# DeepBlender/DeepDenoiser

Measured on AMD Instinct MI355X. Metric: train tiles/sec (128x128x32ch U-Net KPCN), higher is better.
Workload: dtype bf16; 1 GPU; BASELINE config 2: U-Net [64,96,128]x4 + 5x5 KernelPrediction + 3-scale MultiScalePrediction, 32-channel render-pass stack, 128x128 tiles, full training step (fwd+SMAPE loss+bwd+Adam); global_batch=128, parallelism=dp1, hipgraph=True, inputs=resident in HBM

## Files before the change

deepdenoiser_amd/csrc/dd_convt.hip:

```cpp
#include "dd_common.h"

namespace {

struct CtP {
  const void* x; const void* y; const void* w; void* out; float* dw; float* db; const float* bias;
  int ldx, ldy, ldo;
  int cin, cout, cinv, coutv;
  int n_pad, k_pad;
  int B, H, W, tiles_x, tiles_y, nwg;
  int relu;
  int co_off, cout_total;
};

typedef __attribute__((address_space(3))) s16x4_t* ct_tr_ptr;
typedef uint32_t ct_u32x4 __attribute__((ext_vector_type(4)));
typedef uint32_t ct_u32x2 __attribute__((ext_vector_type(2)));

constexpr int CT_T = 8;
constexpr int CT_X_SLICE = CT_T * CT_T * DD_LDS_ROW;
constexpr int CT_X_BYTES = 2 * CT_X_SLICE;
constexpr int CT_Y_BYTES = 4 * CT_T * CT_T * DD_LDS_ROW;
constexpr int CT_BWD_BUF = CT_Y_BYTES + CT_X_BYTES;
constexpr int CT_FWD_BUF = CT_X_BYTES;

__device__ __forceinline__ void ct_dma_1k(const void* gptr, unsigned lds_addr) {
  asm volatile("s_mov_b32 m0, %1\n\ts_nop 0\n\tglobal_load_lds_dwordx4 %0, off" : : "v"(gptr), "s"(lds_addr) : "memory");
}
__device__ __forceinline__ uint4 ct_lds16(unsigned off) {
  const ct_u32x4 v = *reinterpret_cast<const __attribute__((address_space(3))) ct_u32x4*>(off);
  return uint4{v[0], v[1], v[2], v[3]};
}
__device__ __forceinline__ uint2 ct_lds8(unsigned off) {
  const ct_u32x2 v = *reinterpret_cast<const __attribute__((address_space(3))) ct_u32x2*>(off);
  return uint2{v[0], v[1]};
}
__device__ __forceinline__ uint4 ct_tr_pair(unsigned a0, unsigned a1) {
  const s16x4_t lo = __builtin_amdgcn_ds_read_tr16_b64_v4i16(reinterpret_cast<ct_tr_ptr>(a0));
  const s16x4_t hi = __builtin_amdgcn_ds_read_tr16_b64_v4i16(reinterpret_cast<ct_tr_ptr>(a1));
  const uint2 l2 = __builtin_bit_cast(uint2, lo), h2 = __builtin_bit_cast(uint2, hi);
  return uint4{l2.x, l2.y, h2.x, h2.y};
}

struct CtTile { int b, i0, j0; bool live; };
__device__ __forceinline__ CtTile ct_tile(const CtP& a, int tile, int total, int th = CT_T) {
  CtTile t;
  t.live = tile < total;
  const int u = t.live ? tile : 0, per_img = a.tiles_x * a.tiles_y;
  t.b = u / per_img;
  const int rem = u - t.b * per_img, ty = rem / a.tiles_x;
  t.i0 = ty * th; t.j0 = (rem - ty * a.tiles_x) * CT_T;
  return t;
}
template <int TH = CT_T>
__device__ __forceinline__ void ct_dma_x(const CtP& a, const CtTile& t, int xc, unsigned lds, int lane) {
  const int r = lane >> 3, ls = (lane & 7) ^ r;
  const int sx = xc / TH, row = xc % TH, ch = sx * 64 + ls * 8;
  const bool ok = t.live && ch < a.cinv && t.i0 + row < a.H && t.j0 + r < a.W;
  const char* src = reinterpret_cast<const char*>(a.x) + (((long)t.b * a.H + t.i0 + row) * a.W + t.j0 + r) * a.ldx * 2 + ch * 2;
  ct_dma_1k(ok ? src : reinterpret_cast<const char*>(&dd_zero16_v), lds + xc * 1024);
}
template <int NSD>
__device__ __forceinline__ void ct_dma_y(const CtP& a, const CtTile& t, int c, unsigned lds, int lane) {
  const int r = lane >> 3, ls = (lane & 7) ^ r;
  const int sd = c / (32 / NSD), cc = c % (32 / NSD);
  const int row = cc >> 1, col = (cc & 1) * 8 + r, ch = sd * 64 + ls * 8;
  const int gy = 2 * t.i0 + row, gx = 2 * t.j0 + col;
  const bool ok = t.live && ch < a.coutv && gy < 2 * a.H && gx < 2 * a.W;
  const char* src = reinterpret_cast<const char*>(a.y) + (((long)t.b * 2 * a.H + gy) * 2 * a.W + gx) * a.ldy * 2 + (a.co_off + ch) * 2;
  ct_dma_1k(ok ? src : reinterpret_cast<const char*>(&dd_zero16_v), lds + c * 1024);
}

template <typename T, int KC>
__global__ __launch_bounds__(512) void convt_fwd_kernel(const CtP a) {
  extern __shared__ __attribute__((aligned(1024))) char smem[];
  constexpr int NTW = 3;
  const int tid = threadIdx.x, lane = tid & 63, wave = __builtin_amdgcn_readfirstlane(tid >> 6);
  const int li = lane & 15, q = lane >> 4;
  const unsigned lds_base = (unsigned)(uintptr_t)(__attribute__((address_space(3))) char*)smem;
  const int total = a.B * a.tiles_x * a.tiles_y;
  const int ntiles = (4 * a.cout) >> 4;
  const T* Wp = reinterpret_cast<const T*>(a.w);
  const T* zw = reinterpret_cast<const T*>(&dd_zero16_v);
  uint4 wf[NTW][KC];
  float bv[NTW][4];
  int och[NTW], opix[NTW];
  bool nt_ok[NTW];
#pragma unroll
  for (int u = 0; u < NTW; ++u) {
    const int nt = wave + 8 * u;
    nt_ok[u] = nt < ntiles;
    const int nrow = nt * 16 + li;
#pragma unroll
    for (int kc = 0; kc < KC; ++kc) {
      const int k0 = kc * 32 + q * 8;
      const bool ok = nt_ok[u] && nrow < a.n_pad && k0 < a.k_pad;
      wf[u][kc] = *reinterpret_cast<const uint4*>(ok ? Wp + (long)nrow * a.k_pad + k0 : zw);
    }
    const int n4 = nt * 16 + q * 4;
// ... 32 lines not shown
#pragma unroll
        for (int u = 0; u < NTW; ++u) acc[g][u] = mma16<T>(wf[u][kc], f, acc[g][u]);
      }
    const int jj = cur.j0 + (li & 7);
#pragma unroll
    for (int g = 0; g < 4; ++g) {
      const int ii = cur.i0 + 2 * g + (li >> 3);
      const bool ok = ii < a.H && jj < a.W;
      const long p0 = ((long)cur.b * 2 * a.H + 2 * ii) * 2 * a.W + 2 * jj;
#pragma unroll
      for (int u = 0; u < NTW; ++u) {
        f32x4_t v = acc[g][u];
        if (a.relu) { v[0] = fmaxf(v[0], 0.f); v[1] = fmaxf(v[1], 0.f); v[2] = fmaxf(v[2], 0.f); v[3] = fmaxf(v[3], 0.f); }
        uint2 o2;
        o2.x = pack2<T>(v[0], v[1]);
        o2.y = pack2<T>(v[2], v[3]);
        if (ok && nt_ok[u]) *reinterpret_cast<uint2*>(Y + (p0 + opix[u]) * a.ldy + och[u]) = o2;
      }
    }
    cur = nxt;
  }
}

template <typename T> __device__ __forceinline__ void ct_mma_inplace(f32x4_t& acc, const uint4& a, const uint4& b);
template <> __device__ __forceinline__ void ct_mma_inplace<bf16_t>(f32x4_t& acc, const uint4& a, const uint4& b) {
  const ct_u32x4 av = {a.x, a.y, a.z, a.w}, bv = {b.x, b.y, b.z, b.w};
  asm volatile("v_mfma_f32_16x16x32_bf16 %0, %1, %2, %0" : "+v"(acc) : "v"(av), "v"(bv));
}
template <> __device__ __forceinline__ void ct_mma_inplace<f16_t>(f32x4_t& acc, const uint4& a, const uint4& b) {
  const ct_u32x4 av = {a.x, a.y, a.z, a.w}, bv = {b.x, b.y, b.z, b.w};
  asm volatile("v_mfma_f32_16x16x32_f16 %0, %1, %2, %0" : "+v"(acc) : "v"(av), "v"(bv));
}

template <typename T, int NSD, bool MASK, bool ACCUM>
__global__ __launch_bounds__(512) void convt_bwd_kernel(const CtP a) {
  extern __shared__ __attribute__((aligned(1024))) char smem[];
  constexpr int TH = CT_T / NSD, NG = TH / 2, KC = 2 * NSD, JW = 2 * NSD, KS = TH / 4;
  constexpr int Y_SLICE = CT_Y_BYTES / NSD, X_SLICE = CT_T * TH * DD_LDS_ROW, BUF = CT_Y_BYTES + 2 * X_SLICE;
  const int tid = threadIdx.x, lane = tid & 63, wave = __builtin_amdgcn_readfirstlane(tid >> 6);
  const int li = lane & 15, q = lane >> 4;
  const unsigned lds_base = (unsigned)(uintptr_t)(__attribute__((address_space(3))) char*)smem;
  const int total = a.B * a.tiles_x * a.tiles_y;

  const bool d_active = wave * 16 < a.cin;
  uint4 wf[4][KC];
  {
    const T* Wd = reinterpret_cast<const T*>(a.w);
    const T* zw = reinterpret_cast<const T*>(&dd_zero16_v);
    const int ci_row = wave * 16 + li;
#pragma unroll
    for (int t = 0; t < 4; ++t)
#pragma unroll
      for (int kc = 0; kc < KC; ++kc) {
        const int k0 = kc * 32 + q * 8;
        const bool ok = ci_row < a.n_pad && k0 < a.coutv && a.co_off + k0 < a.k_pad;
        wf[t][kc] = *reinterpret_cast<const uint4*>(ok ? Wd + ((long)t * a.n_pad + ci_row) * a.k_pad + a.co_off + k0 : zw);
      }
  }
  unsigned db[4];
#pragma unroll
  for (int t = 0; t < 4; ++t) {
    const int pd = (2 * (li >> 3) + (t >> 1)) * 16 + 2 * (li & 7) + (t & 1);
    db[t] = lds_base + pd * DD_LDS_ROW + ((q ^ (pd & 7)) << 4);
  }
  const unsigned mb = lds_base + CT_Y_BYTES + (wave >> 2) * X_SLICE + li * DD_LDS_ROW + ((((wave & 3) * 2 + (q >> 1)) ^ (li & 7)) << 4) + (q & 1) * 8;
  const int c4 = wave * 16 + q * 4;
  T* __restrict__ DX = reinterpret_cast<T*>(a.out);

  const int tw = wave & 3, h = wave >> 2;
  const bool w_active = h * JW * 16 < a.cout;
  const int nci = (a.cin + 15) >> 4;
  unsigned yb[2], xb[2];
  {
    const int t16 = lane & 15, gq = lane >> 4, sub = t16 & 3;
#pragma unroll
    for (int hh = 0; hh < 2; ++hh) {
      const int col = (t16 >> 2) + 4 * hh;
      const int pd = (2 * gq + (tw >> 1)) * 16 + 2 * col + (tw & 1), px = gq * 8 + col;
      yb[hh] = lds_base + ((h * JW) >> 2) * Y_SLICE + pd * DD_LDS_ROW + (((((h * JW) & 3) * 2 + (sub >> 1)) ^ (pd & 7)) << 4) + (sub & 1) * 8;
      xb[hh] = lds_base + CT_Y_BYTES + px * DD_LDS_ROW + (((sub >> 1) ^ (px & 7)) << 4) + (sub & 1) * 8;
    }
  }
  f32x4_t wacc[JW][8];
#pragma unroll
  for (int j = 0; j < JW; ++j)
#pragma unroll
    for (int i = 0; i < 8; ++i) wacc[j][i] = f32x4_t{0.f, 0.f, 0.f, 0.f};
  float bsum[JW];
#pragma unroll
  for (int j = 0; j < JW; ++j) bsum[j] = 0.f;

  auto dma_tile = [&](const CtTile& t, unsigned buf) {
#pragma unroll
    for (int k = 0; k < 4; ++k) ct_dma_y<NSD>(a, t, k * 8 + wave, buf, lane);
    ct_dma_x<TH>(a, t, wave, buf + CT_Y_BYTES, lane);
    if (NSD == 1) ct_dma_x<TH>(a, t, wave + 8, buf + CT_Y_BYTES, lane);
  };
  constexpr int NPW = 5 + (NSD == 1 ? 1 : 0);
  CtTile cur = ct_tile(a, blockIdx.x, total, TH);
  dma_tile(cur, lds_base);
  int sel = 0;
  for (int tile = blockIdx.x; tile < total; tile += a.nwg, sel ^= 1) {
    __builtin_amdgcn_s_waitcnt(0x0F70);
    __syncthreads();
    const CtTile nxt = ct_tile(a, tile + a.nwg, total, TH);
    const int jj = cur.j0 + (li & 7);
    const bool ch_ok = c4 < a.cinv && jj < a.W;
    ct_u32x2 oldr[NG];
    if (ACCUM) {
#pragma unroll
      for (int g = 0; g < NG; ++g) {
        const int ii = cur.i0 + 2 * g + (li >> 3);
        const bool ok = d_active && ch_ok && ii < a.H;
        const void* op = ok ? static_cast<const void*>(DX + (((long)cur.b * a.H + ii) * a.W + jj) * a.ldo + c4) : static_cast<const void*>(&dd_zero16_v);
        asm volatile("global_load_dwordx2 %0, %1, off ; dd_accum_request" : "=v"(oldr[g]) : "v"(op) : "memory");
      }
    }
    dma_tile(nxt, lds_base + (sel ^ 1) * BUF);
    const unsigned bt = sel * BUF;
    if (d_active) {
      f32x4_t acc[NG];
      uint2 mv[NG], oldv[NG];
#pragma unroll
      for (int g = 0; g < NG; ++g) {
        acc[g] = f32x4_t{0.f, 0.f, 0.f, 0.f};
        if (MASK) mv[g] = ct_lds8(bt + mb + g * 16 * DD_LDS_ROW);
        oldv[g] = uint2{0u, 0u};
      }
#pragma unroll
      for (int t = 0; t < 4; ++t)
#pragma unroll
        for (int kc = 0; kc < KC; ++kc)
#pragma unroll
          for (int g = 0; g < NG; ++g) {
            const uint4 f = ct_lds16(bt + (db[t] ^ ((kc & 1) << 6)) + (kc >> 1) * Y_SLICE + g * 64 * DD_LDS_ROW);
            acc[g] = mma16<T>(wf[t][kc], f, acc[g]);
          }
      if (ACCUM) {
        static_assert(NG == 4 || NG == 2, "the wait below names every request register");
        if constexpr (NG == 4) {
          if constexpr (NPW == 6) asm volatile("s_waitcnt vmcnt(6) ; dd_accum_wait" : "+v"(oldr[0]), "+v"(oldr[1]), "+v"(oldr[2]), "+v"(oldr[3]));
          else asm volatile("s_waitcnt vmcnt(5) ; dd_accum_wait" : "+v"(oldr[0]), "+v"(oldr[1]), "+v"(oldr[2]), "+v"(oldr[3]));
        } else {
          if constexpr (NPW == 6) asm volatile("s_waitcnt vmcnt(6) ; dd_accum_wait" : "+v"(oldr[0]), "+v"(oldr[1]));
          else asm volatile("s_waitcnt vmcnt(5) ; dd_accum_wait" : "+v"(oldr[0]), "+v"(oldr[1]));
        }
#pragma unroll
        for (int g = 0; g < NG; ++g) oldv[g] = uint2{oldr[g][0], oldr[g][1]};
      }
#pragma unroll
      for (int g = 0; g < NG; ++g) {
        const int ii = cur.i0 + 2 * g + (li >> 3);
        uint2 o2;
        o2.x = pack2<T>(acc[g][0], acc[g][1]);
        o2.y = pack2<T>(acc[g][2], acc[g][3]);
        if (MASK) { o2.x = mask_bf16x2(o2.x, mv[g].x); o2.y = mask_bf16x2(o2.y, mv[g].y); }
        if (ACCUM) {
          float f8[8], g8[8];
          unpack8t<T>(uint4{o2.x, o2.y, 0u, 0u}, f8);
          unpack8t<T>(uint4{oldv[g].x, oldv[g].y, 0u, 0u}, g8);
          o2.x = pack2<T>(f8[0] + g8[0], f8[1] + g8[1]);
          o2.y = pack2<T>(f8[2] + g8[2], f8[3] + g8[3]);
        }
        if (ch_ok && ii < a.H) *reinterpret_cast<uint2*>(DX + (((long)cur.b * a.H + ii) * a.W + jj) * a.ldo + c4) = o2;
      }
    }
    if (w_active) {
#pragma unroll
      for (int s = 0; s < KS; ++s) {
        uint4 yf[JW];
#pragma unroll
        for (int j = 0; j < JW; ++j)
          yf[j] = ct_tr_pair(bt + (yb[0] ^ (j << 5)) + s * 128 * DD_LDS_ROW, bt + (yb[1] ^ (j << 5)) + s * 128 * DD_LDS_ROW);
#pragma unroll
        for (int i = 0; i < 8; ++i) {
          if (i >= nci) continue;
          const uint4 xf = ct_tr_pair(bt + (xb[0] ^ ((i & 3) << 5)) + (i >> 2) * X_SLICE + s * 32 * DD_LDS_ROW,
                                      bt + (xb[1] ^ ((i & 3) << 5)) + (i >> 2) * X_SLICE + s * 32 * DD_LDS_ROW);
#pragma unroll
          for (int j = 0; j < JW; ++j) ct_mma_inplace<T>(wacc[j][i], yf[j], xf);
        }
        if (a.db) {
#pragma unroll
          for (int j = 0; j < JW; ++j) {
            float f[8];
            unpack8t<T>(yf[j], f);
            bsum[j] += ((f[0] + f[1]) + (f[2] + f[3])) + ((f[4] + f[5]) + (f[6] + f[7]));
          }
        }
      }
    }
    cur = nxt;
  }
  asm volatile("s_nop 15\n\ts_nop 15" ::: "memory");
  dd_det_wait();
  if (w_active) {
#pragma unroll
    for (int j = 0; j < JW; ++j)
#pragma unroll
      for (int i = 0; i < 8; ++i) {
        const int ci = i * 16 + li;
        if (i >= nci || ci >= a.cin) continue;
#pragma unroll
        for (int e = 0; e < 4; ++e) {
          const int co = (h * JW + j) * 16 + q * 4 + e;
          if (co < a.cout) atomicAdd(a.dw + ((long)tw * a.cout_total + a.co_off + co) * a.cin + ci, wacc[j][i][e]);
// ... 19 lines not shown

static int ct_cus() {
  return dd_device_cus();
}

template <typename K>
static void ct_launch(K kernel, const CtP& p, size_t lds, hipStream_t stream) {
  dd_det_sync();
  dd_allow_max_lds(reinterpret_cast<const void*>(kernel));
  hipLaunchKernelGGL(kernel, dim3((unsigned)p.nwg), dim3(512), lds, stream, p);
}

static int ct_fill(CtP& p, const dd_convt_args* a, bool bwd) {
  const int th = CT_T;
  DD_REQUIRE(a && a->x && a->y && a->w, "dd_convt2x2: null pointer");
  DD_REQUIRE(a->dtype == DD_BF16 || a->dtype == DD_F16, "dd_convt2x2: dtype %d (bf16 / f16 storage only; f32 takes dd_conv_igemm / dd_conv_wgrad)", a->dtype);
  DD_REQUIRE(a->cin > 0 && a->cin <= 128 && a->cout > 0 && a->cout <= (bwd ? 128 : 96) && a->cout % 16 == 0,
             "dd_convt2x2: cin=%d cout=%d (cin <= 128; cout a multiple of 16, <= 96 forward / 128 backward)", a->cin, a->cout);
  const int cinv = (a->cin + 7) / 8 * 8, coutv = (a->cout + 7) / 8 * 8;
  DD_REQUIRE(a->ld_x % 8 == 0 && a->ld_y % 8 == 0 && cinv <= a->ld_x && coutv <= a->ld_y, "dd_convt2x2: ld_x=%d ld_y=%d must be multiples of 8 covering the channels", a->ld_x, a->ld_y);
  DD_REQUIRE(((uintptr_t)a->x % 16) == 0 && ((uintptr_t)a->y % 16) == 0 && ((uintptr_t)a->w % 16) == 0, "dd_convt2x2: x / y / w must be 16-byte aligned");
  DD_REQUIRE(a->B > 0 && a->H > 0 && a->W > 0 && (long)a->B * a->H * a->W * 4 < (1L << 31), "dd_convt2x2: empty or oversized grid");
  p.x = a->x; p.y = a->y; p.w = a->w; p.ldx = a->ld_x; p.ldy = a->ld_y;
  p.cin = a->cin; p.cout = a->cout; p.cinv = cinv; p.coutv = coutv; p.n_pad = a->n_pad; p.k_pad = a->k_pad;
  p.B = a->B; p.H = a->H; p.W = a->W;
  p.tiles_x = dd_ceil_div(a->W, CT_T); p.tiles_y = dd_ceil_div(a->H, th);
  const long total = (long)a->B * p.tiles_x * p.tiles_y;
  p.nwg = (int)(total < ct_cus() ? total : ct_cus());
  p.relu = a->relu;
  p.co_off = 0; p.cout_total = a->cout;
  return DD_OK;
}

}

extern "C" int dd_convt2x2_fwd(const dd_convt_args* a, dd_stream stream) {
  CtP p;
  if (int rc = ct_fill(p, a, false)) return rc;
  DD_REQUIRE(a->n_pad >= 4 * a->cout && a->k_pad >= a->cin && a->k_pad % 32 == 0 && a->k_pad <= 128, "dd_convt2x2_fwd: packed weights [n_pad=%d][k_pad=%d]", a->n_pad, a->k_pad);
  p.out = const_cast<void*>(a->y); p.bias = a->bias; p.dw = nullptr; p.db = nullptr; p.ldo = 0;
  hipStream_t s = reinterpret_cast<hipStream_t>(stream);
  const size_t lds = 2 * (size_t)CT_FWD_BUF;
  const int kc = a->k_pad / 32;
#define CT_FWD(T)                                                            \
  switch (kc) {                                                              \
    case 1: ct_launch(convt_fwd_kernel<T, 1>, p, lds, s); break;             \
    case 2: ct_launch(convt_fwd_kernel<T, 2>, p, lds, s); break;             \
    case 3: ct_launch(convt_fwd_kernel<T, 3>, p, lds, s); break;             \
    default: ct_launch(convt_fwd_kernel<T, 4>, p, lds, s); break;            \
  }
  if (a->dtype == DD_BF16) { CT_FWD(bf16_t) } else { CT_FWD(f16_t) }
#undef CT_FWD
  DD_LAUNCH_CHECK();
  return DD_OK;
}

extern "C" int dd_convt2x2_bwd(const dd_convt_args* a, dd_stream stream) {
  CtP p;
  if (int rc = ct_fill(p, a, true)) return rc;
  DD_REQUIRE(a->dx && a->dw, "dd_convt2x2_bwd: null gradient pointer");
  DD_REQUIRE(a->n_pad >= a->cin && a->k_pad >= a->cout && a->k_pad % 8 == 0, "dd_convt2x2_bwd: packed weights [4][n_pad=%d][k_pad=%d]", a->n_pad, a->k_pad);
  const int cinv = (a->cin + 7) / 8 * 8;
  DD_REQUIRE(a->ld_dx % 4 == 0 && cinv <= a->ld_dx && ((uintptr_t)a->dx % 8) == 0, "dd_convt2x2_bwd: ld_dx=%d / dx alignment", a->ld_dx);
  p.out = a->dx; p.ldo = a->ld_dx; p.dw = a->dw; p.db = a->db; p.bias = nullptr;
  hipStream_t s = reinterpret_cast<hipStream_t>(stream);
  const size_t lds = 2 * (size_t)CT_BWD_BUF;
#define CT_BWD_N(T, N, ACC)                                                                                \
  if (a->use_mask) { if (ACC) ct_launch(convt_bwd_kernel<T, N, true, true>, p, lds, s); else ct_launch(convt_bwd_kernel<T, N, true, false>, p, lds, s); } \
  else { if (ACC) ct_launch(convt_bwd_kernel<T, N, false, true>, p, lds, s); else ct_launch(convt_bwd_kernel<T, N, false, false>, p, lds, s); }
  for (int co_off = 0; co_off < a->cout; co_off += 64) {
    const int cb = a->cout - co_off < 64 ? a->cout - co_off : 64;
    p.co_off = co_off; p.cout = cb; p.coutv = (cb + 7) / 8 * 8; p.cout_total = a->cout;
    const bool acc = a->accumulate || co_off > 0;
    if (a->dtype == DD_BF16) { CT_BWD_N(bf16_t, 1, acc) } else { CT_BWD_N(f16_t, 1, acc) }
  }
#undef CT_BWD_N
  DD_LAUNCH_CHECK();
  return DD_OK;
}
```

deepdenoiser_amd/_lib.py:

```python

import ctypes as C
import os

_HERE = os.path.dirname(os.path.abspath(__file__))
LIB_PATH = os.environ.get("DD_LIB", os.path.join(_HERE, "libdd_hip.so"))

DD_F32, DD_BF16, DD_F16 = 0, 1, 2
IN_RELU, OUT_RELU, ACCUM, PIXSHUF, GATHER2X2 = 1, 2, 4, 8, 16
MAX_FEATURES, MAX_COMBINED = 32, 8
METRIC_SOURCES = MAX_FEATURES + MAX_COMBINED + 1

SYMBOLS = (
    "dd_version", "dd_last_error", "dd_pack_weights", "dd_pack_weights_batched", "dd_conv_igemm", "dd_conv_wgrad", "dd_colsum", "dd_colsum_segments",
    "dd_maxpool_fwd", "dd_maxpool_bwd", "dd_avgpool", "dd_prepare_feature", "dd_gather_input",
    "dd_kpcn_fwd", "dd_kpcn_bwd", "dd_kpcn_hidden_fwd", "dd_kpcn_hidden_bwd", "dd_compose_pack", "dd_compose_blend_fwd", "dd_compose_blend_bwd",
    "dd_compose_unpack_bwd", "dd_invert_std_fwd", "dd_invert_std_bwd", "dd_loss_head", "dd_adam_step",
    "dd_stitch", "dd_recombine", "dd_probe_tr16", "dd_masked_add", "dd_zero_stuff", "dd_zero_unstuff", "dd_convert_channels",
    "dd_augment", "dd_loss_mask_sums", "dd_crc32c", "dd_extract_tiles", "dd_compose_net_fwd", "dd_compose_net_bwd",
    "dd_kpcn_head_fwd", "dd_kpcn_head_bwd", "dd_kpcn_head_bwd_multi", "dd_assemble_input", "dd_assemble_input_frames", "dd_conv3x3_bwd", "dd_conv3x3_bwd_multi", "dd_convt2x2_fwd", "dd_convt2x2_bwd", "dd_conv3x3_ks",
    "dd_conv_pw_count", "dd_wgrad_pw_count", "dd_space_to_depth2", "dd_convt3_wgrad", "dd_compose_stream_plan", "dd_compose_bwd_scratch_bytes",
    "dd_loss_msssim_scratch_bytes", "dd_loss_msssim_fwd", "dd_loss_msssim_bwd", "dd_loss_msssim_values",
    "dd_loss_metrics_scratch_bytes", "dd_loss_metrics", "dd_loss_head_path_count",
)


class ConvT3WgradArgs(C.Structure):
    _fields_ = [("s", C.c_void_p), ("lds", C.c_int), ("cout", C.c_int), ("cp", C.c_int),
                ("x", C.c_void_p), ("ldx", C.c_int), ("cin", C.c_int),
                ("dk", C.c_void_p),
                ("B", C.c_int), ("H", C.c_int), ("W", C.c_int), ("dtype", C.c_int)]


class ConvArgs(C.Structure):
    _fields_ = [("x", C.c_void_p), ("ldx", C.c_int), ("cin", C.c_int),
                ("wp", C.c_void_p), ("k_pad", C.c_int), ("n_pad", C.c_int),
                ("bias", C.c_void_p), ("nbias", C.c_int),
                ("res", C.c_void_p), ("ldres", C.c_int),
                ("mask", C.c_void_p), ("ldmask", C.c_int),
                ("y", C.c_void_p), ("ldy", C.c_int), ("n", C.c_int),
                ("B", C.c_int), ("H", C.c_int), ("W", C.c_int),
                ("taps", C.c_int), ("flags", C.c_int), ("dtype", C.c_int)]


class WgradArgs(C.Structure):
    _fields_ = [("p", C.c_void_p), ("ldp", C.c_int), ("m", C.c_int),
                ("q", C.c_void_p), ("ldq", C.c_int), ("n", C.c_int),
                ("out", C.c_void_p), ("bias_out", C.c_void_p), ("bias_mode", C.c_int),
                ("B", C.c_int), ("H", C.c_int), ("W", C.c_int),
                ("taps", C.c_int), ("flags", C.c_int), ("dtype", C.c_int), ("ksplit", C.c_int),
                ("stack_blocks", C.c_int), ("stack_width", C.c_int), ("stack_m0", C.c_int),
                ("stack_out", C.c_void_p * 8), ("stack_bias", C.c_void_p * 8)]

# ... 142 lines not shown
                           % (got.split("src=")[-1], want))


def source_hash():
    return load().dd_version().decode().split("src=")[-1]


def load():
    global _lib
    if _lib is not None:
        return _lib
    import torch
    if not os.path.exists(LIB_PATH):
        raise RuntimeError("libdd_hip.so is not built (%s missing): run `python -m deepdenoiser_amd.build`. "
                           "There is no CPU/PyTorch fallback for the hot path." % LIB_PATH)
    lib = C.CDLL(LIB_PATH)
    missing = [s for s in SYMBOLS if not hasattr(lib, s)]
    if missing:
        raise RuntimeError("libdd_hip.so lacks symbols %s: rebuild it" % missing)
    lib.dd_version.restype = C.c_char_p
    lib.dd_last_error.restype = C.c_char_p
    _check_source_hash(lib)
    for s in SYMBOLS[2:]:
        getattr(lib, s).restype = C.c_int
    vp, i, l, f = C.c_void_p, C.c_int, C.c_long, C.c_float
    lib.dd_pack_weights.argtypes = [vp, vp, i, i, i, i, i, i, l, l, l, i, vp]
    lib.dd_pack_weights_batched.argtypes = [vp, i, i, vp]
    lib.dd_conv_igemm.argtypes = [C.POINTER(ConvArgs), vp]
    lib.dd_conv_wgrad.argtypes = [C.POINTER(WgradArgs), vp]
    lib.dd_conv3x3_bwd.argtypes = [C.POINTER(ConvBwdArgs), vp]
    lib.dd_conv3x3_bwd_multi.argtypes = [C.POINTER(ConvBwdArgs), i, vp]
    lib.dd_convt2x2_fwd.argtypes = [C.POINTER(ConvTArgs), vp]
    lib.dd_convt2x2_bwd.argtypes = [C.POINTER(ConvTArgs), vp]
    lib.dd_conv3x3_ks.argtypes = [C.POINTER(ConvKsArgs), vp]
    lib.dd_space_to_depth2.argtypes = [vp, i, vp, i, i, i, i, i, i, i, vp]
    lib.dd_convt3_wgrad.argtypes = [C.POINTER(ConvT3WgradArgs), vp]
    lib.dd_conv_pw_count.argtypes = []
    lib.dd_conv_pw_count.restype = C.c_long
    lib.dd_wgrad_pw_count.argtypes = []
    lib.dd_wgrad_pw_count.restype = C.c_long
    lib.dd_colsum.argtypes = [vp, i, i, l, vp, i, vp]
    lib.dd_colsum_segments.argtypes = [vp, i, i, l, i, vp, i, vp, i, vp]
    lib.dd_maxpool_fwd.argtypes = [vp, i, vp, i, vp, i, i, i, i, i, i, i, i, vp]
    lib.dd_maxpool_bwd.argtypes = [vp, i, vp, vp, i, vp, i, i, i, i, i, i, i, i, i, vp]
    lib.dd_avgpool.argtypes = [vp, i, vp, i, i, i, i, i, i, vp]
    lib.dd_prepare_feature.argtypes = [vp, i, vp, i, C.POINTER(FeatureParams), i, i, i, vp]
    lib.dd_gather_input.argtypes = [vp, i, i, vp, i, i, i, i, i, i, vp]
    lib.dd_kpcn_fwd.argtypes = [vp, i, vp, i, vp, i, i, i, i, i, i, vp]
    lib.dd_kpcn_bwd.argtypes = [vp, i, vp, i, vp, i, vp, i, i, i, i, i, i, i, vp]
    lib.dd_kpcn_hidden_fwd.argtypes = [vp, i, vp, i, i, vp, i, vp, vp, i, i, i, i, i, i, vp]
    lib.dd_kpcn_hidden_bwd.argtypes = [vp, i, vp, i, i, vp, i, vp, vp, i, vp, i, i, i, i, i, i, i, vp]
    lib.dd_compose_pack.argtypes = [vp, i, vp, i, vp, i, i, i, i, i, i, vp]
    lib.dd_compose_blend_fwd.argtypes = [vp, i, vp, i, vp, i, vp, i, i, i, i, i, vp]
    lib.dd_compose_blend_bwd.argtypes = [vp, i, vp, i, vp, i, vp, i, vp, i, i, vp, i, vp, i, i, i, i, i, i, vp]
    lib.dd_compose_unpack_bwd.argtypes = [vp, i, vp, i, vp, i, i, i, i, i, vp]
    lib.dd_invert_std_fwd.argtypes = [vp, vp, l, i, f, f, vp]
    lib.dd_invert_std_bwd.argtypes = [vp, vp, vp, l, i, f, f, vp]
    lib.dd_loss_head.argtypes = [C.POINTER(LossDesc), i, i, i, vp, f, vp]
    lib.dd_loss_head_path_count.argtypes = [i]
    lib.dd_loss_head_path_count.restype = C.c_long
    lib.dd_loss_msssim_scratch_bytes.argtypes = [i, i, i, i]
    lib.dd_loss_msssim_scratch_bytes.restype = C.c_long
    lib.dd_loss_msssim_fwd.argtypes = [C.POINTER(MsSsimDesc), i, i, i, vp, vp, vp]
    lib.dd_loss_msssim_bwd.argtypes = [C.POINTER(MsSsimDesc), i, i, i, vp, f, vp]
    lib.dd_loss_msssim_values.argtypes = [C.POINTER(MsSsimDesc), i, i, i, vp, vp, vp]
    lib.dd_loss_metrics_scratch_bytes.argtypes = [i, i, i]
# ... 32 lines not shown
```

include/dd_hip.h:

```cpp
#ifndef DD_HIP_H
#define DD_HIP_H

#include <stddef.h>
#include <stdint.h>

#ifdef __cplusplus
extern "C" {
#endif

typedef void* dd_stream;

enum dd_dtype { DD_F32 = 0, DD_BF16 = 1, DD_F16 = 2 };

enum dd_status {
  DD_OK = 0,
  DD_ERR_INVALID = -1,
  DD_ERR_LAUNCH = -2
};

enum dd_conv_flags {
  DD_IN_RELU = 1,
  DD_OUT_RELU = 2,
  DD_ACCUM = 4,
  DD_PIXSHUF = 8,
// ... 29 lines not shown
  float* out;
  float* bias_out; int bias_mode;
  int B, H, W;
  int taps; int flags; int dtype;
  int ksplit;
  int stack_blocks; int stack_width; int stack_m0;
  float* stack_out[8]; float* stack_bias[8];
} dd_wgrad_args;
int dd_conv_wgrad(const dd_wgrad_args* a, dd_stream stream);

typedef struct {
  const void* dy; int ld_dy; int cout;
  const void* x; int ld_x; int cin;
  const void* wd; int n_pad; int k_pad;
  void* dx; int ld_dx;
  float* dw; float* db;
  int B, H, W;
  int use_mask; int accumulate; int dtype;
} dd_conv_bwd_args;
int dd_conv3x3_bwd(const dd_conv_bwd_args* a, dd_stream stream);
int dd_conv3x3_bwd_multi(const dd_conv_bwd_args* a, int n, dd_stream stream);

typedef struct {
  const void* x; int ld_x; int cin;
  void* y; int ld_y; int cout;
  const void* w; int n_pad; int k_pad;
  const float* bias; int relu;
  void* dx; int ld_dx; float* dw; float* db; int use_mask; int accumulate;
  int B, H, W;
  int dtype;
} dd_convt_args;
int dd_convt2x2_fwd(const dd_convt_args* a, dd_stream stream);
int dd_convt2x2_bwd(const dd_convt_args* a, dd_stream stream);

typedef struct {
  const void* x; int ldx; int cin;
  const void* wp; int n_pad; int k_pad;
  const float* bias; int nbias;
  void* y; int ldy;
  int n0; int n;
  int B, H, W;
  int mode; int flags; int dtype;
  const void* mask; int ldmask;
} dd_conv_ks_args;
int dd_conv3x3_ks(const dd_conv_ks_args* a, dd_stream stream);

int dd_colsum(const void* x, int ld, int c, long rows, float* out, int dtype, dd_stream stream);
int dd_colsum_segments(const void* x, int ld, int c, long rows_per_segment, int n_segments, float* out, int out_ld, const int* out_row,
                       int dtype, dd_stream stream);

int dd_maxpool_fwd(const void* x, int ldx, void* y, int ldy, uint8_t* idx, int C, int B, int H, int W,
                   int pool, int stride, int relu_mask, int dtype, dd_stream stream);
int dd_maxpool_bwd(const void* dy, int lddy, const uint8_t* idx, void* dx, int lddx, const void* mask, int ldmask,
                   int C, int B, int H, int W, int pool, int stride, int accumulate, int dtype, dd_stream stream);

int dd_avgpool(const float* x, int ldx, float* y, int ldy, int C, int B, int H, int W, int f, dd_stream stream);

typedef struct {
  int use_log1p; float mean; float inv_std;
  int use_variance; int variance_before; int mode_neighbor; int relative; int compress; float epsilon;
} dd_feature_params;
int dd_prepare_feature(const float* src, int cs, float* dst, int ldd, const dd_feature_params* fp, int B, int H, int W, dd_stream stream);

typedef struct { const float* src; int pixel_stride; int batch_stride_pixels; int nch; int dst_ch; } dd_gather_entry;
int dd_gather_input(const dd_gather_entry* table, int n_tuples, int n_entries, void* dst, int ld, int c_pad,
                    int B, int H, int W, int dtype, dd_stream stream);
// ... 185 lines not shown
```

Baseline: 15340 tiles/s.

## Handle 65-96 output channels in one transposed-conv backward launch

Adds a three-chunk variant of the transposed-conv backward kernel. It stages 96 dy channels in LDS, with an extra half-size dy buffer and a new address mapping, so layers with up to 96 output channels run in a single launch instead of two 64-channel passes. This removes the second pass's re-read of x and dx, along with its read-modify-write accumulate, at the cost of more LDS per block and possibly lower occupancy. The wait counts and the DMA layout are reworked to match.

```diff
diff --git a/deepdenoiser_amd/csrc/dd_convt.hip b/deepdenoiser_amd/csrc/dd_convt.hip
--- a/deepdenoiser_amd/csrc/dd_convt.hip
+++ b/deepdenoiser_amd/csrc/dd_convt.hip
@@ -20,7 +20,7 @@
 constexpr int CT_X_SLICE = CT_T * CT_T * DD_LDS_ROW;
 constexpr int CT_X_BYTES = 2 * CT_X_SLICE;
 constexpr int CT_Y_BYTES = 4 * CT_T * CT_T * DD_LDS_ROW;
-constexpr int CT_BWD_BUF = CT_Y_BYTES + CT_X_BYTES;
+constexpr int CT_Y2_BYTES = CT_Y_BYTES / 2;
 constexpr int CT_FWD_BUF = CT_X_BYTES;
 
 __device__ __forceinline__ void ct_dma_1k(const void* gptr, unsigned lds_addr) {
@@ -59,11 +59,11 @@
   const char* src = reinterpret_cast<const char*>(a.x) + (((long)t.b * a.H + t.i0 + row) * a.W + t.j0 + r) * a.ldx * 2 + ch * 2;
   ct_dma_1k(ok ? src : reinterpret_cast<const char*>(&dd_zero16_v), lds + xc * 1024);
 }
-template <int NSD>
+template <bool HI>
 __device__ __forceinline__ void ct_dma_y(const CtP& a, const CtTile& t, int c, unsigned lds, int lane) {
   const int r = lane >> 3, ls = (lane & 7) ^ r;
-  const int sd = c / (32 / NSD), cc = c % (32 / NSD);
-  const int row = cc >> 1, col = (cc & 1) * 8 + r, ch = sd * 64 + ls * 8;
+  const int pd = HI ? c * 8 + r + (ls >> 2) * 128 : c * 8 + r;
+  const int row = pd >> 4, col = pd & 15, ch = HI ? 64 + (ls & 3) * 8 : ls * 8;
   const int gy = 2 * t.i0 + row, gx = 2 * t.j0 + col;
   const bool ok = t.live && ch < a.coutv && gy < 2 * a.H && gx < 2 * a.W;
   const char* src = reinterpret_cast<const char*>(a.y) + (((long)t.b * 2 * a.H + gy) * 2 * a.W + gx) * a.ldy * 2 + (a.co_off + ch) * 2;
@@ -162,11 +162,12 @@
   asm volatile("v_mfma_f32_16x16x32_f16 %0, %1, %2, %0" : "+v"(acc) : "v"(av), "v"(bv));
 }
 
-template <typename T, int NSD, bool MASK, bool ACCUM>
+template <typename T, int NCO, bool MASK, bool ACCUM>
 __global__ __launch_bounds__(512) void convt_bwd_kernel(const CtP a) {
   extern __shared__ __attribute__((aligned(1024))) char smem[];
-  constexpr int TH = CT_T / NSD, NG = TH / 2, KC = 2 * NSD, JW = 2 * NSD, KS = TH / 4;
-  constexpr int Y_SLICE = CT_Y_BYTES / NSD, X_SLICE = CT_T * TH * DD_LDS_ROW, BUF = CT_Y_BYTES + 2 * X_SLICE;
+  static_assert(NCO == 2 || NCO == 3, "two or three 32-channel chunks of dy");
+  constexpr int TH = CT_T, NG = TH / 2, KC = NCO, JW = NCO, KS = TH / 4;
+  constexpr int Y_BYTES = CT_Y_BYTES + (NCO == 3 ? CT_Y2_BYTES : 0), X_SLICE = CT_X_SLICE, BUF = Y_BYTES + CT_X_BYTES;
   const int tid = threadIdx.x, lane = tid & 63, wave = __builtin_amdgcn_readfirstlane(tid >> 6);
   const int li = lane & 15, q = lane >> 4;
   const unsigned lds_base = (unsigned)(uintptr_t)(__attribute__((address_space(3))) char*)smem;
@@ -193,7 +194,7 @@
     const int pd = (2 * (li >> 3) + (t >> 1)) * 16 + 2 * (li & 7) + (t & 1);
     db[t] = lds_base + pd * DD_LDS_ROW + ((q ^ (pd & 7)) << 4);
   }
-  const unsigned mb = lds_base + CT_Y_BYTES + (wave >> 2) * X_SLICE + li * DD_LDS_ROW + ((((wave & 3) * 2 + (q >> 1)) ^ (li & 7)) << 4) + (q & 1) * 8;
+  const unsigned mb = lds_base + Y_BYTES + (wave >> 2) * X_SLICE + li * DD_LDS_ROW + ((((wave & 3) * 2 + (q >> 1)) ^ (li & 7)) << 4) + (q & 1) * 8;
   const int c4 = wave * 16 + q * 4;
   T* __restrict__ DX = reinterpret_cast<T*>(a.out);
 
@@ -207,8 +208,8 @@
     for (int hh = 0; hh < 2; ++hh) {
       const int col = (t16 >> 2) + 4 * hh;
       const int pd = (2 * gq + (tw >> 1)) * 16 + 2 * col + (tw & 1), px = gq * 8 + col;
-      yb[hh] = lds_base + ((h * JW) >> 2) * Y_SLICE + pd * DD_LDS_ROW + (((((h * JW) & 3) * 2 + (sub >> 1)) ^ (pd & 7)) << 4) + (sub & 1) * 8;
-      xb[hh] = lds_base + CT_Y_BYTES + px * DD_LDS_ROW + (((sub >> 1) ^ (px & 7)) << 4) + (sub & 1) * 8;
+      yb[hh] = lds_base + pd * DD_LDS_ROW + ((((NCO == 2 ? h * JW * 2 : 0) + (sub >> 1)) ^ (pd & 7)) << 4) + (sub & 1) * 8;
+      xb[hh] = lds_base + Y_BYTES + px * DD_LDS_ROW + (((sub >> 1) ^ (px & 7)) << 4) + (sub & 1) * 8;
     }
   }
   f32x4_t wacc[JW][8];
@@ -220,13 +221,23 @@
 #pragma unroll
   for (int j = 0; j < JW; ++j) bsum[j] = 0.f;
 
+  auto y_tile = [&](unsigned ybase, int j, int s) -> unsigned {
+    if constexpr (NCO == 2) return (ybase ^ (j << 5)) + s * 128 * DD_LDS_ROW;
+    const int ot = h * JW + j;
+    const bool lo = ot < 4;
+    return (ybase ^ (((ot & 3) << 5) | (lo ? 0 : s << 6))) + (lo ? s * 128 * DD_LDS_ROW : CT_Y_BYTES);
+  };
   auto dma_tile = [&](const CtTile& t, unsigned buf) {
 #pragma unroll
-    for (int k = 0; k < 4; ++k) ct_dma_y<NSD>(a, t, k * 8 + wave, buf, lane);
-    ct_dma_x<TH>(a, t, wave, buf + CT_Y_BYTES, lane);
-    if (NSD == 1) ct_dma_x<TH>(a, t, wave + 8, buf + CT_Y_BYTES, lane);
+    for (int k = 0; k < 4; ++k) ct_dma_y<false>(a, t, k * 8 + wave, buf, lane);
+    if constexpr (NCO == 3) {
+      ct_dma_y<true>(a, t, wave, buf + CT_Y_BYTES, lane);
+      ct_dma_y<true>(a, t, wave + 8, buf + CT_Y_BYTES, lane);
+    }
+    ct_dma_x<TH>(a, t, wave, buf + Y_BYTES, lane);
+    ct_dma_x<TH>(a, t, wave + 8, buf + Y_BYTES, lane);
   };
-  constexpr int NPW = 5 + (NSD == 1 ? 1 : 0);
+  constexpr int NPW = NCO == 3 ? 8 : 6;
   CtTile cur = ct_tile(a, blockIdx.x, total, TH);
   dma_tile(cur, lds_base);
   int sel = 0;
@@ -263,18 +274,14 @@
         for (int kc = 0; kc < KC; ++kc)
 #pragma unroll
           for (int g = 0; g < NG; ++g) {
-            const uint4 f = ct_lds16(bt + (db[t] ^ ((kc & 1) << 6)) + (kc >> 1) * Y_SLICE + g * 64 * DD_LDS_ROW);
+            const uint4 f = kc < 2 ? ct_lds16(bt + (db[t] ^ (kc << 6)) + g * 64 * DD_LDS_ROW)
+                                   : ct_lds16(bt + (db[t] ^ ((g >> 1) << 6)) + CT_Y_BYTES + (g & 1) * 64 * DD_LDS_ROW);
             acc[g] = mma16<T>(wf[t][kc], f, acc[g]);
           }
       if (ACCUM) {
-        static_assert(NG == 4 || NG == 2, "the wait below names every request register");
-        if constexpr (NG == 4) {
-          if constexpr (NPW == 6) asm volatile("s_waitcnt vmcnt(6) ; dd_accum_wait" : "+v"(oldr[0]), "+v"(oldr[1]), "+v"(oldr[2]), "+v"(oldr[3]));
-          else asm volatile("s_waitcnt vmcnt(5) ; dd_accum_wait" : "+v"(oldr[0]), "+v"(oldr[1]), "+v"(oldr[2]), "+v"(oldr[3]));
-        } else {
-          if constexpr (NPW == 6) asm volatile("s_waitcnt vmcnt(6) ; dd_accum_wait" : "+v"(oldr[0]), "+v"(oldr[1]));
-          else asm volatile("s_waitcnt vmcnt(5) ; dd_accum_wait" : "+v"(oldr[0]), "+v"(oldr[1]));
-        }
+        static_assert(NG == 4 && (NPW == 6 || NPW == 8), "the wait below names every request register and counts the DMA pieces behind them");
+        if constexpr (NPW == 6) asm volatile("s_waitcnt vmcnt(6) ; dd_accum_wait" : "+v"(oldr[0]), "+v"(oldr[1]), "+v"(oldr[2]), "+v"(oldr[3]));
+        else asm volatile("s_waitcnt vmcnt(8) ; dd_accum_wait" : "+v"(oldr[0]), "+v"(oldr[1]), "+v"(oldr[2]), "+v"(oldr[3]));
 #pragma unroll
         for (int g = 0; g < NG; ++g) oldv[g] = uint2{oldr[g][0], oldr[g][1]};
       }
@@ -300,8 +307,7 @@
       for (int s = 0; s < KS; ++s) {
         uint4 yf[JW];
 #pragma unroll
-        for (int j = 0; j < JW; ++j)
-          yf[j] = ct_tr_pair(bt + (yb[0] ^ (j << 5)) + s * 128 * DD_LDS_ROW, bt + (yb[1] ^ (j << 5)) + s * 128 * DD_LDS_ROW);
+        for (int j = 0; j < JW; ++j) yf[j] = ct_tr_pair(bt + y_tile(yb[0], j, s), bt + y_tile(yb[1], j, s));
 #pragma unroll
         for (int i = 0; i < 8; ++i) {
           if (i >= nci) continue;
@@ -419,15 +425,26 @@
   DD_REQUIRE(a->ld_dx % 4 == 0 && cinv <= a->ld_dx && ((uintptr_t)a->dx % 8) == 0, "dd_convt2x2_bwd: ld_dx=%d / dx alignment", a->ld_dx);
   p.out = a->dx; p.ldo = a->ld_dx; p.dw = a->dw; p.db = a->db; p.bias = nullptr;
   hipStream_t s = reinterpret_cast<hipStream_t>(stream);
-  const size_t lds = 2 * (size_t)CT_BWD_BUF;
 #define CT_BWD_N(T, N, ACC)                                                                                \
   if (a->use_mask) { if (ACC) ct_launch(convt_bwd_kernel<T, N, true, true>, p, lds, s); else ct_launch(convt_bwd_kernel<T, N, true, false>, p, lds, s); } \
   else { if (ACC) ct_launch(convt_bwd_kernel<T, N, false, true>, p, lds, s); else ct_launch(convt_bwd_kernel<T, N, false, false>, p, lds, s); }
-  for (int co_off = 0; co_off < a->cout; co_off += 64) {
-    const int cb = a->cout - co_off < 64 ? a->cout - co_off : 64;
-    p.co_off = co_off; p.cout = cb; p.coutv = (cb + 7) / 8 * 8; p.cout_total = a->cout;
-    const bool acc = a->accumulate || co_off > 0;
-    if (a->dtype == DD_BF16) { CT_BWD_N(bf16_t, 1, acc) } else { CT_BWD_N(f16_t, 1, acc) }
+  if (a->cout <= 96) {
+    const bool acc = a->accumulate != 0;
+    if (a->cout <= 64) {
+      const size_t lds = 2 * (size_t)(CT_Y_BYTES + CT_X_BYTES);
+      if (a->dtype == DD_BF16) { CT_BWD_N(bf16_t, 2, acc) } else { CT_BWD_N(f16_t, 2, acc) }
+    } else {
+      const size_t lds = 2 * (size_t)(CT_Y_BYTES + CT_Y2_BYTES + CT_X_BYTES);
+      if (a->dtype == DD_BF16) { CT_BWD_N(bf16_t, 3, acc) } else { CT_BWD_N(f16_t, 3, acc) }
+    }
+  } else {
+    const size_t lds = 2 * (size_t)(CT_Y_BYTES + CT_X_BYTES);
+    for (int co_off = 0; co_off < a->cout; co_off += 64) {
+      const int cb = a->cout - co_off < 64 ? a->cout - co_off : 64;
+      p.co_off = co_off; p.cout = cb; p.coutv = (cb + 7) / 8 * 8; p.cout_total = a->cout;
+      const bool acc = a->accumulate || co_off > 0;
+      if (a->dtype == DD_BF16) { CT_BWD_N(bf16_t, 2, acc) } else { CT_BWD_N(f16_t, 2, acc) }
+    }
   }
 #undef CT_BWD_N
   DD_LAUNCH_CHECK();
```

Measured after the change: 15440 tiles/s (median of 6 runs). No clear change (+0.6%).

## Fuse wide transposed-conv backward into one launch with half-height tiles

Applied to the files above, without the earlier changes.

For transposed 2x2 convolutions whose output channel count lies between 64 and 96, the backward pass now runs as a single launch over all output channels instead of two launches split at 64 channels. It uses half-height spatial tiles so the 96-channel dy block fits in two LDS slices. The kernel gains an NCT template parameter for the number of output-channel tiles, with precomputed per-tile LDS offsets. This drops the second launch and the re-read and re-accumulation of dx that the split required. In exchange, each tile carries more per-wave weight fragments and accumulators, which raises register pressure, and the smaller tiles add more per-tile DMA overhead.

```diff
diff --git a/deepdenoiser_amd/_lib.py b/deepdenoiser_amd/_lib.py
--- a/deepdenoiser_amd/_lib.py
+++ b/deepdenoiser_amd/_lib.py
@@ -17,7 +17,7 @@
     "dd_compose_unpack_bwd", "dd_invert_std_fwd", "dd_invert_std_bwd", "dd_loss_head", "dd_adam_step",
     "dd_stitch", "dd_recombine", "dd_probe_tr16", "dd_masked_add", "dd_zero_stuff", "dd_zero_unstuff", "dd_convert_channels",
     "dd_augment", "dd_loss_mask_sums", "dd_crc32c", "dd_extract_tiles", "dd_compose_net_fwd", "dd_compose_net_bwd",
-    "dd_kpcn_head_fwd", "dd_kpcn_head_bwd", "dd_kpcn_head_bwd_multi", "dd_assemble_input", "dd_assemble_input_frames", "dd_conv3x3_bwd", "dd_conv3x3_bwd_multi", "dd_convt2x2_fwd", "dd_convt2x2_bwd", "dd_conv3x3_ks",
+    "dd_kpcn_head_fwd", "dd_kpcn_head_bwd", "dd_kpcn_head_bwd_multi", "dd_assemble_input", "dd_assemble_input_frames", "dd_conv3x3_bwd", "dd_conv3x3_bwd_multi", "dd_convt2x2_fwd", "dd_convt2x2_bwd", "dd_convt2x2_bwd_plan", "dd_conv3x3_ks",
     "dd_conv_pw_count", "dd_wgrad_pw_count", "dd_space_to_depth2", "dd_convt3_wgrad", "dd_compose_stream_plan", "dd_compose_bwd_scratch_bytes",
     "dd_loss_msssim_scratch_bytes", "dd_loss_msssim_fwd", "dd_loss_msssim_bwd", "dd_loss_msssim_values",
     "dd_loss_metrics_scratch_bytes", "dd_loss_metrics", "dd_loss_head_path_count",
@@ -226,6 +226,7 @@
     lib.dd_conv3x3_bwd_multi.argtypes = [C.POINTER(ConvBwdArgs), i, vp]
     lib.dd_convt2x2_fwd.argtypes = [C.POINTER(ConvTArgs), vp]
     lib.dd_convt2x2_bwd.argtypes = [C.POINTER(ConvTArgs), vp]
+    lib.dd_convt2x2_bwd_plan.argtypes = [C.POINTER(ConvTArgs), C.POINTER(C.c_int), C.POINTER(C.c_int)]
     lib.dd_conv3x3_ks.argtypes = [C.POINTER(ConvKsArgs), vp]
     lib.dd_space_to_depth2.argtypes = [vp, i, vp, i, i, i, i, i, i, i, vp]
     lib.dd_convt3_wgrad.argtypes = [C.POINTER(ConvT3WgradArgs), vp]
diff --git a/deepdenoiser_amd/csrc/dd_convt.hip b/deepdenoiser_amd/csrc/dd_convt.hip
--- a/deepdenoiser_amd/csrc/dd_convt.hip
+++ b/deepdenoiser_amd/csrc/dd_convt.hip
@@ -162,10 +162,24 @@
   asm volatile("v_mfma_f32_16x16x32_f16 %0, %1, %2, %0" : "+v"(acc) : "v"(av), "v"(bv));
 }
 
-template <typename T, int NSD, bool MASK, bool ACCUM>
+template <int NPW, int NG>
+__device__ __forceinline__ void ct_accum_wait(ct_u32x2 (&oldr)[NG]) {
+  static_assert((NG == 4 || NG == 2) && (NPW == 6 || NPW == 5), "one asm statement per (pieces, request registers)");
+  if constexpr (NG == 4) {
+    if constexpr (NPW == 6) asm volatile("s_waitcnt vmcnt(6) ; dd_accum_wait" : "+v"(oldr[0]), "+v"(oldr[1]), "+v"(oldr[2]), "+v"(oldr[3]));
+    else asm volatile("s_waitcnt vmcnt(5) ; dd_accum_wait" : "+v"(oldr[0]), "+v"(oldr[1]), "+v"(oldr[2]), "+v"(oldr[3]));
+  } else {
+    if constexpr (NPW == 6) asm volatile("s_waitcnt vmcnt(6) ; dd_accum_wait" : "+v"(oldr[0]), "+v"(oldr[1]));
+    else asm volatile("s_waitcnt vmcnt(5) ; dd_accum_wait" : "+v"(oldr[0]), "+v"(oldr[1]));
+  }
+}
+
+template <typename T, int NSD, int NCT, bool MASK, bool ACCUM>
 __global__ __launch_bounds__(512) void convt_bwd_kernel(const CtP a) {
   extern __shared__ __attribute__((aligned(1024))) char smem[];
-  constexpr int TH = CT_T / NSD, NG = TH / 2, KC = 2 * NSD, JW = 2 * NSD, KS = TH / 4;
+  static_assert(NCT % 2 == 0 && NCT > 4 * (NSD - 1) && NCT <= 4 * NSD, "the output tiles must need exactly NSD slices of dy");
+  constexpr int TH = CT_T / NSD, NG = TH / 2, KC = (NCT + 1) / 2, JW = NCT / 2, KS = TH / 4;
+  constexpr bool JX = (JW & (JW - 1)) == 0;
   constexpr int Y_SLICE = CT_Y_BYTES / NSD, X_SLICE = CT_T * TH * DD_LDS_ROW, BUF = CT_Y_BYTES + 2 * X_SLICE;
   const int tid = threadIdx.x, lane = tid & 63, wave = __builtin_amdgcn_readfirstlane(tid >> 6);
   const int li = lane & 15, q = lane >> 4;
@@ -207,9 +221,17 @@
     for (int hh = 0; hh < 2; ++hh) {
       const int col = (t16 >> 2) + 4 * hh;
       const int pd = (2 * gq + (tw >> 1)) * 16 + 2 * col + (tw & 1), px = gq * 8 + col;
-      yb[hh] = lds_base + ((h * JW) >> 2) * Y_SLICE + pd * DD_LDS_ROW + (((((h * JW) & 3) * 2 + (sub >> 1)) ^ (pd & 7)) << 4) + (sub & 1) * 8;
+      const int ot0 = JX ? h * JW : 0;
+      yb[hh] = lds_base + (ot0 >> 2) * Y_SLICE + pd * DD_LDS_ROW + ((((ot0 & 3) * 2 + (sub >> 1)) ^ (pd & 7)) << 4) + (sub & 1) * 8;
       xb[hh] = lds_base + CT_Y_BYTES + px * DD_LDS_ROW + (((sub >> 1) ^ (px & 7)) << 4) + (sub & 1) * 8;
     }
+  }
+  unsigned yx[JW], ys[JW];
+#pragma unroll
+  for (int j = 0; j < JW; ++j) {
+    const int ot = JX ? j : h * JW + j;
+    yx[j] = (unsigned)(ot & 3) << 5;
+    ys[j] = (unsigned)(ot >> 2) * Y_SLICE;
   }
   f32x4_t wacc[JW][8];
 #pragma unroll
@@ -226,7 +248,8 @@
     ct_dma_x<TH>(a, t, wave, buf + CT_Y_BYTES, lane);
     if (NSD == 1) ct_dma_x<TH>(a, t, wave + 8, buf + CT_Y_BYTES, lane);
   };
-  constexpr int NPW = 5 + (NSD == 1 ? 1 : 0);
+  constexpr int NPW = 4 + 2 * TH / 8;
+  static_assert(NPW == (NSD == 1 ? 6 : 5), "the vmcnt of dd_accum_wait below is the number of DMA pieces a wave issues behind the request");
   CtTile cur = ct_tile(a, blockIdx.x, total, TH);
   dma_tile(cur, lds_base);
   int sel = 0;
@@ -248,15 +271,17 @@
     }
     dma_tile(nxt, lds_base + (sel ^ 1) * BUF);
     const unsigned bt = sel * BUF;
+    f32x4_t acc[NG];
+    uint2 mv[NG], oldv[NG];
+#pragma unroll
+    for (int g = 0; g < NG; ++g) {
+      acc[g] = f32x4_t{0.f, 0.f, 0.f, 0.f};
+      mv[g] = oldv[g] = uint2{0u, 0u};
+    }
     if (d_active) {
-      f32x4_t acc[NG];
-      uint2 mv[NG], oldv[NG];
-#pragma unroll
-      for (int g = 0; g < NG; ++g) {
-        acc[g] = f32x4_t{0.f, 0.f, 0.f, 0.f};
+#pragma unroll
+      for (int g = 0; g < NG; ++g)
         if (MASK) mv[g] = ct_lds8(bt + mb + g * 16 * DD_LDS_ROW);
-        oldv[g] = uint2{0u, 0u};
-      }
 #pragma unroll
       for (int t = 0; t < 4; ++t)
 #pragma unroll
@@ -266,18 +291,13 @@
             const uint4 f = ct_lds16(bt + (db[t] ^ ((kc & 1) << 6)) + (kc >> 1) * Y_SLICE + g * 64 * DD_LDS_ROW);
             acc[g] = mma16<T>(wf[t][kc], f, acc[g]);
           }
-      if (ACCUM) {
-        static_assert(NG == 4 || NG == 2, "the wait below names every request register");
-        if constexpr (NG == 4) {
-          if constexpr (NPW == 6) asm volatile("s_waitcnt vmcnt(6) ; dd_accum_wait" : "+v"(oldr[0]), "+v"(oldr[1]), "+v"(oldr[2]), "+v"(oldr[3]));
-          else asm volatile("s_waitcnt vmcnt(5) ; dd_accum_wait" : "+v"(oldr[0]), "+v"(oldr[1]), "+v"(oldr[2]), "+v"(oldr[3]));
-        } else {
-          if constexpr (NPW == 6) asm volatile("s_waitcnt vmcnt(6) ; dd_accum_wait" : "+v"(oldr[0]), "+v"(oldr[1]));
-          else asm volatile("s_waitcnt vmcnt(5) ; dd_accum_wait" : "+v"(oldr[0]), "+v"(oldr[1]));
-        }
-#pragma unroll
-        for (int g = 0; g < NG; ++g) oldv[g] = uint2{oldr[g][0], oldr[g][1]};
-      }
+    }
+    if (ACCUM) {
+      ct_accum_wait<NPW>(oldr);
+#pragma unroll
+      for (int g = 0; g < NG; ++g) oldv[g] = uint2{oldr[g][0], oldr[g][1]};
+    }
+    if (d_active) {
 #pragma unroll
       for (int g = 0; g < NG; ++g) {
         const int ii = cur.i0 + 2 * g + (li >> 3);
@@ -301,7 +321,7 @@
         uint4 yf[JW];
 #pragma unroll
         for (int j = 0; j < JW; ++j)
-          yf[j] = ct_tr_pair(bt + (yb[0] ^ (j << 5)) + s * 128 * DD_LDS_ROW, bt + (yb[1] ^ (j << 5)) + s * 128 * DD_LDS_ROW);
+          yf[j] = ct_tr_pair(bt + (yb[0] ^ yx[j]) + ys[j] + s * 128 * DD_LDS_ROW, bt + (yb[1] ^ yx[j]) + ys[j] + s * 128 * DD_LDS_ROW);
 #pragma unroll
         for (int i = 0; i < 8; ++i) {
           if (i >= nci) continue;
@@ -387,6 +407,20 @@
   return DD_OK;
 }
 
+static void ct_bwd_plan(int cout, int* launches, int* tile_h) {
+  const bool wide = cout > 64 && cout <= 96;
+  *launches = wide ? 1 : (cout + 63) / 64;
+  *tile_h = wide ? CT_T / 2 : CT_T;
+}
+
+}
+
+extern "C" int dd_convt2x2_bwd_plan(const dd_convt_args* a, int* launches, int* tile_h) {
+  DD_REQUIRE(a && launches && tile_h, "dd_convt2x2_bwd_plan: null pointer");
+  DD_REQUIRE(a->cin > 0 && a->cin <= 128 && a->cout > 0 && a->cout <= 128 && a->cout % 16 == 0,
+             "dd_convt2x2_bwd_plan: cin=%d cout=%d (cin <= 128; cout a multiple of 16, <= 128)", a->cin, a->cout);
+  ct_bwd_plan(a->cout, launches, tile_h);
+  return DD_OK;
 }
 
 extern "C" int dd_convt2x2_fwd(const dd_convt_args* a, dd_stream stream) {
@@ -419,15 +453,26 @@
   DD_REQUIRE(a->ld_dx % 4 == 0 && cinv <= a->ld_dx && ((uintptr_t)a->dx % 8) == 0, "dd_convt2x2_bwd: ld_dx=%d / dx alignment", a->ld_dx);
   p.out = a->dx; p.ldo = a->ld_dx; p.dw = a->dw; p.db = a->db; p.bias = nullptr;
   hipStream_t s = reinterpret_cast<hipStream_t>(stream);
-  const size_t lds = 2 * (size_t)CT_BWD_BUF;
-#define CT_BWD_N(T, N, ACC)                                                                                \
-  if (a->use_mask) { if (ACC) ct_launch(convt_bwd_kernel<T, N, true, true>, p, lds, s); else ct_launch(convt_bwd_kernel<T, N, true, false>, p, lds, s); } \
-  else { if (ACC) ct_launch(convt_bwd_kernel<T, N, false, true>, p, lds, s); else ct_launch(convt_bwd_kernel<T, N, false, false>, p, lds, s); }
-  for (int co_off = 0; co_off < a->cout; co_off += 64) {
-    const int cb = a->cout - co_off < 64 ? a->cout - co_off : 64;
-    p.co_off = co_off; p.cout = cb; p.coutv = (cb + 7) / 8 * 8; p.cout_total = a->cout;
-    const bool acc = a->accumulate || co_off > 0;
-    if (a->dtype == DD_BF16) { CT_BWD_N(bf16_t, 1, acc) } else { CT_BWD_N(f16_t, 1, acc) }
+#define CT_BWD_N(T, NSD, NCT, ACC, LDS)                                                                     \
+  if (a->use_mask) { if (ACC) ct_launch(convt_bwd_kernel<T, NSD, NCT, true, true>, p, LDS, s); else ct_launch(convt_bwd_kernel<T, NSD, NCT, true, false>, p, LDS, s); } \
+  else { if (ACC) ct_launch(convt_bwd_kernel<T, NSD, NCT, false, true>, p, LDS, s); else ct_launch(convt_bwd_kernel<T, NSD, NCT, false, false>, p, LDS, s); }
+  int launches, tile_h;
+  ct_bwd_plan(a->cout, &launches, &tile_h);
+  if (tile_h != CT_T) {
+    p.tiles_y = dd_ceil_div(a->H, tile_h);
+    const long total = (long)a->B * p.tiles_x * p.tiles_y;
+    p.nwg = (int)(total < ct_cus() ? total : ct_cus());
+    const size_t lds = 2 * ((size_t)CT_Y_BYTES + 2 * (size_t)CT_T * tile_h * DD_LDS_ROW);
+    const bool acc = a->accumulate != 0;
+    if (a->dtype == DD_BF16) { CT_BWD_N(bf16_t, 2, 6, acc, lds) } else { CT_BWD_N(f16_t, 2, 6, acc, lds) }
+  } else {
+    const size_t lds = 2 * (size_t)CT_BWD_BUF;
+    for (int co_off = 0; co_off < a->cout; co_off += 64) {
+      const int cb = a->cout - co_off < 64 ? a->cout - co_off : 64;
+      p.co_off = co_off; p.cout = cb; p.coutv = (cb + 7) / 8 * 8; p.cout_total = a->cout;
+      const bool acc = a->accumulate || co_off > 0;
+      if (a->dtype == DD_BF16) { CT_BWD_N(bf16_t, 1, 4, acc, lds) } else { CT_BWD_N(f16_t, 1, 4, acc, lds) }
+    }
   }
 #undef CT_BWD_N
   DD_LAUNCH_CHECK();
diff --git a/include/dd_hip.h b/include/dd_hip.h
--- a/include/dd_hip.h
+++ b/include/dd_hip.h
@@ -85,6 +85,7 @@
 } dd_convt_args;
 int dd_convt2x2_fwd(const dd_convt_args* a, dd_stream stream);
 int dd_convt2x2_bwd(const dd_convt_args* a, dd_stream stream);
+int dd_convt2x2_bwd_plan(const dd_convt_args* a, int* launches, int* tile_h);
 
 typedef struct {
   const void* x; int ldx; int cin;
```

Result: no change. 16080 tiles/s before, 16190 tiles/s after (median of 6 runs) (+0.7%).
